# HKPolyU-UAV/bluerov2

Measured on AMD Instinct MI355X. Metric: NMPC RTI solves/s (N=20, 12 states / 4 inputs), batch 4096 per GPU, higher is better.
Workload: dtype f64; 1 GPU; BASELINE.json configs[1]: batch=4096 independent BlueROV2 NMPC instances per GPU, N=20, Ts=0.05 s, circle reference window advancing one row per step, per-instance x0 noise (seed 1), nominal parameters, default options (qp_early_exit=1: exact equality-constrained shortcut when no bound is active); batch_per_gpu=4096, N=20, parallelism=single GPU

## Files before the change

### bluerov2_amd/csrc/nmpc_api.hip

```cpp
#include <hip/hip_runtime.h>

#include <algorithm>
#include <cstddef>
#include <cstdio>
#include <cstdlib>
#include <cmath>
#include <cstring>
#include <string>
#include <atomic>
#include <chrono>
#include <vector>

#include "host_common.hpp"
#include "nmpc_device.hpp"
#include "select_device.hpp"
#include "wrench_source.hpp"

using namespace brov;

#define kTickMailboxMaxBatch 64

static thread_local std::string g_err;
extern "C" const char* brov_last_error(void) { return g_err.c_str(); }

// ... 69 lines not shown
    WrenchSource wr;
    bool cand_set = false;
    int cand_kind = 0;
    bool dump_lin = false;
    int* lines = nullptr;
    DeviceAllocs mem;
    hipStream_t last_stream = nullptr;
    bool timing = false;
    hipEvent_t ev[3] = {nullptr, nullptr, nullptr};
    bool ev_valid = false;
    int last_family = 0;
    int cus = 256;
    double* ws = nullptr;
    int32_t* counter = nullptr;
    unsigned win_count = 0;
    int win_blocks = 0, win_L = 0;
    double* ws_split = nullptr;
    int alt_blocks = 0, alt_L = 0;
    int prep_path = 0;
    unsigned long long* dbg = nullptr;
    std::vector<double> ts_host;
    double W0_host[16] = {0};
    bool has_W0 = false;
    double* tsv = nullptr;
    double* wst = nullptr;
    int32_t* sched = nullptr;
    unsigned sched_tick = 0;
    TickChannel tick;
    bool pit_ran = false;
    int32_t* pit_done = nullptr;
    DevKnobs k;
};

static int env_int(const char* name, int dflt) { const char* v = getenv(name); return v ? atoi(v) : dflt; }
static DevKnobs read_knobs() {
    DevKnobs k;
    k.robust_pivot = env_int("BROV_ROBUST_PIVOT", 1);
    if (const char* v = getenv("BROV_ROBUST_KKT_MAX")) k.robust_kkt_max = atof(v);
    k.partial_refactor = env_int("BROV_PARTIAL_REFACTOR", 1) != 0;
    k.mail_early = env_int("BROV_DEV_NO_EARLY_RECORD", 0) == 0;
    k.split_resident = env_int("BROV_SPLIT_RESIDENT", 1) != 0;
    k.pit = env_int("BROV_PIT", 1);
    k.split_parallel = env_int("BROV_SPLIT_PARALLEL", 1) != 0;
    k.pit_try = env_int("BROV_PIT_TRY", 1) != 0;
    k.pit_light = env_int("BROV_PIT_LIGHT", 1) != 0;
    k.tick_mailbox = env_int("BROV_TICK_MAILBOX", 1) != 0;
    k.tick_bulk = env_int("BROV_TICK_BULK", 1) != 0;
    k.tick_zerocopy = env_int("BROV_TICK_ZEROCOPY", 1) != 0;
    k.sched = env_int("BROV_SCHED", 1) != 0;
    k.force_windowed = env_int("BROV_DEV_FORCE_WINDOWED", 0) != 0;
    k.fused_waves = env_int("BROV_DEV_FUSED_WAVES", 0);
    k.lds_pad = env_int("BROV_DEV_LDS_PAD", 0);
    k.closed_loop_fused = env_int("BROV_CLOSED_LOOP_FUSED", 1) != 0;
    k.tick_breakdown = env_int("BROV_TICK_BREAKDOWN", 0) != 0;
    k.no_resident = env_int("BROV_DEV_NO_RESIDENT", 0) != 0;
    k.win_blocks = env_int("BROV_DEV_WIN_BLOCKS", 0);
    k.pit_rounds = env_int("BROV_PIT_ROUNDS", 1) != 0;
    k.win_long = env_int("BROV_DEV_WIN_LONG", 0) != 0;
    return k;
}
extern "C" int brov_dev_reload_knobs(brov_solver* s) {
    if (!s) return BROV_ERR_ARG;
    const DevKnobs at_create = s->k;
    s->k = read_knobs();
    s->k.force_windowed = at_create.force_windowed; s->k.no_resident = at_create.no_resident;
    s->k.win_blocks = at_create.win_blocks; s->k.pit_rounds = at_create.pit_rounds;
    return BROV_OK;
}

extern "C" void brov_default_opts(brov_opts* o, int N, double Ts) {
    static const double W[16] = {300, 480, 200, 10, 10, 200, 40, 40, 10, 10, 10, 10, 1, 1, 0.1, 0.05};
    std::memset(o, 0, sizeof(*o));
    o->N = N;
    o->Ts = Ts;
    for (int j = 0; j < 16; j++) o->W[j] = W[j];
    for (int j = 0; j < 12; j++) o->We[j] = W[j];
    for (int j = 0; j < 4; j++) { o->lbu[j] = -50.0; o->ubu[j] = 50.0; }
    o->qp_iter_max = 50;
    o->qp_tol_mu = 1e-7;
    o->qp_tol_stat = 1e-9;
    o->qp_early_exit = 1;
    o->kernel_path = BROV_PATH_AUTO;
    o->on_failure = BROV_ON_FAILURE_RESTART;
}

static const char* opts_problem(const brov_opts* o) {
    if (o->N < 1 || o->N > BROV_MAX_N) return "N out of range";
    if (!(o->Ts > 0.0) || !(o->Ts < 1e6)) return "Ts must be positive and finite";
    if (o->kernel_path < 0 || o->kernel_path > 2) return "kernel_path must be BROV_PATH_AUTO / _STREAMING / _FUSED";
    if (o->on_failure < 0 || o->on_failure > 1) return "on_failure must be BROV_ON_FAILURE_KEEP / _RESTART";
    for (int j = 0; j < 16; j++)
        if (!(o->W[j] >= 0.0) || !(o->W[j] < 1e300)) return "stage weights must be finite and >= 0";
    for (int j = 12; j < 16; j++)
        if (!(o->W[j] > 0.0)) return "input weights W[12..15] must be > 0 (strictly convex QP)";
    for (int j = 0; j < 12; j++)
        if (!(o->We[j] >= 0.0) || !(o->We[j] < 1e300)) return "terminal weights must be finite and >= 0";
    for (int j = 0; j < 4; j++)
        if (!(o->lbu[j] < o->ubu[j]) || !(o->lbu[j] > -1e300) || !(o->ubu[j] < 1e300)) return "input bounds need lbu < ubu, both finite";
    if (o->qp_iter_max < 1) return "qp_iter_max must be >= 1";
    if (!(o->qp_tol_mu > 0.0) || !(o->qp_tol_stat > 0.0)) return "qp tolerances must be > 0";
    return nullptr;
}

static void invalidate_preparation(brov_solver* s) { if (s && s->prep_path == 2) s->prep_path = 3; }
static void forget_traj_window(brov_solver* s) { s->yref_view = nullptr; s->traj_line = -1; }
static bool serves_fused(const brov_solver* s) { return fused_supported(s->N) && !s->k.force_windowed; }
static bool serves_windowed_ticks(const brov_solver* s) { return s->ws != nullptr && !windowed_is_resident(s->win_L) && s->alt_L == 0; }

static bool general_grid(const brov_solver* s) { return !s->ts_host.empty() || s->has_W0; }
static int upload_grid(brov_solver* s) {
    if (!general_grid(s)) return BROV_OK;
    const int N = s->N;
    if (!s->tsv) {
        if (int rc = s->mem.alloc(&s->tsv, (size_t)N, g_err)) return rc;
        if (int rc = s->mem.alloc(&s->wst, (size_t)(N + 1) * 16, g_err)) return rc;
    }
    std::vector<double> ts(N), w((size_t)(N + 1) * 16, 0.0);
    for (int i = 0; i < N; i++) {
        ts[i] = s->ts_host.empty() ? s->opts.Ts : s->ts_host[i];
// ... 529 lines not shown
enum { FAM_STREAMING = 0, FAM_FUSED, FAM_WINDOWED };
struct SolvePlan {
    int family = FAM_STREAMING;
    bool split_ok = false;
    int rti_split = 0;
    double* ws = nullptr;
    int64_t ws_stride = 0;
    int win_L = 0, win_blocks = 0;
    int pit = 0, pit_blocks = 0;
    int prep_path = 1;
};
static SolvePlan plan_solve(const brov_solver* s, int rti_phase) {
    SolvePlan p;
    const bool lds = s->opts.kernel_path != BROV_PATH_STREAMING, fused_h = serves_fused(s);
    const bool may_split = lds && !s->dump_lin && s->k.split_resident;
    const bool split_fused = may_split && fused_h && s->ws_split != nullptr;
    p.split_ok = split_fused || (may_split && !fused_h && s->ws != nullptr && windowed_is_resident(s->win_L) && s->win_blocks == s->B);
    const bool split = p.split_ok && (rti_phase == 1 || (rti_phase == 2 && s->prep_path == 2));
    p.prep_path = split ? 2 : 1;
    p.ws = s->ws; p.win_L = s->win_L; p.win_blocks = s->win_blocks;
    if (split && split_fused) { p.ws = s->ws_split; p.win_L = s->N; p.win_blocks = s->B; }
    p.ws_stride = p.win_L ? (int64_t)windowed_ws_doubles(s->N, p.win_L) : 0;
    if (!lds || (rti_phase != 0 && !split)) return p;
    if (fused_h && !split) { p.family = FAM_FUSED; return p; }
    if (!p.ws) return p;
    p.family = FAM_WINDOWED;
    p.rti_split = rti_phase;
    p.pit_blocks = p.win_blocks;
    bool pit = false;
    if (s->k.pit && rti_phase == 2) {
        pit = s->k.split_parallel && pit_supported(s->N, p.win_L);
    } else if (s->k.pit && rti_phase == 0 && !s->dump_lin) {
        if (s->alt_L) {
            p.win_L = s->alt_L; p.win_blocks = s->alt_blocks; p.ws_stride = (int64_t)windowed_ws_doubles(s->N, s->alt_L);
            p.pit_blocks = s->B;
        }
        pit = pit_supported(s->N, p.win_L);
    }
    p.pit = pit ? s->k.pit : 0;
    return p;
}

static DevParams make_params(const brov_solver* s, const SolvePlan& plan, const LaunchInputs* in = nullptr) {
    static const LaunchInputs none;
    if (!in) in = &none;
    DevParams P;
    std::memset(&P, 0, sizeof P);
    P.B = s->B; P.N = s->N;
    P.qp_iter_max = s->opts.qp_iter_max; P.early_exit = s->opts.qp_early_exit;
    P.on_failure = s->opts.on_failure; P.dump_lin = s->dump_lin ? 1 : 0;
    P.robust_kkt_max = s->k.robust_kkt_max;
    P.robust_pivot = s->k.robust_pivot;
    P.partial_refactor = s->k.partial_refactor;
    P.Ts = s->opts.Ts; P.tol_mu = s->opts.qp_tol_mu; P.tol_stat = s->opts.qp_tol_stat;
    for (int j = 0; j < 16; j++) P.W[j] = s->opts.W[j];
    for (int j = 0; j < 12; j++) P.We[j] = s->opts.We[j];
    for (int j = 0; j < 4; j++) { P.lbu[j] = s->opts.lbu[j]; P.ubu[j] = s->opts.ubu[j]; }
    P.x0 = in->x0 ? in->x0 : s->x0;
    P.yref = in->yref ? in->yref : (s->yref_shared ? shared_window(s) : s->yref);
    P.yref_stride = s->yref_shared ? 0 : (int64_t)(s->N + 1) * 16;
    P.par = in->par ? in->par : s->par;
    P.par_rp = s->dist6 ? s->par_rp : nullptr;
    P.tsv = general_grid(s) ? s->tsv : nullptr;
    P.sched = s->k.sched ? s->sched : nullptr;
    P.sched_stride = sched_buffer_ints_host(s->B);
    P.sched_r = (int)(s->sched_tick % 3); P.sched_w = (int)((s->sched_tick + 1) % 3); P.sched_z = (int)((s->sched_tick + 2) % 3);
    P.wst = general_grid(s) ? s->wst : nullptr;
    P.x = s->x; P.u = s->u; P.pi = s->pi; P.lam = s->lam;
    P.BA = s->BA; P.bvec = s->bvec; P.kktp = s->kktp;
    P.Ks = s->Ks; P.Kt = s->Kt; P.Mt = s->Mt; P.Pb = s->Pb; P.kff = s->kff; P.vhat = s->vhat; P.ipm = s->ipm;
    P.dxb = s->dxb; P.cst = s->cst; P.res = s->res;
    P.mail = in->mail; P.mail_flag = in->mail_flag; P.mail_seq = in->mail_seq;
    P.mail_early = s->k.mail_early;
    P.counter = s->counter + 32 * (s->win_count & 1u);
    P.counter_next = s->counter + 32 * ((s->win_count + 1u) & 1u);
    P.ws = plan.ws; P.ws_stride = plan.ws_stride; P.win_L = plan.win_L; P.win_blocks = plan.win_blocks;
    P.rti_split = plan.rti_split; P.pit_blocks = plan.pit_blocks;
    if (plan.pit) { P.pit = plan.pit; P.pit_done = s->pit_done; P.pit_try = s->k.pit_try; P.pit_light = s->k.pit_light; }
    P.dbg = s->dbg;
    return P;
}
static void launch_lds(brov_solver* s, const DevParams& P, int family, hipStream_t st) {
    if (family == FAM_FUSED) launch_fused(P, st, s->k);
    else { launch_windowed(P, st, s->k); s->win_count++; }
    s->pit_ran = P.pit != 0;
    s->last_family = family;
    s->last_stream = st;
}
static void time_mark(brov_solver* s, int k, hipStream_t st) {
    if (s->timing) { hipEventRecord(s->ev[k], st); s->ev_valid = s->ev_valid || k == 2; }
}
struct PlantInLaunch { double dt; int substeps; double *xlog, *ulog; };
static int launch_ticks(brov_solver* s, int family, int n, int64_t row_stride_doubles, int32_t* status_log, const PlantInLaunch* plant,
                        hipStream_t st) {
    if (int rc = order_behind_last(s, st)) return rc;
    DevParams P = make_params(s, plan_solve(s, 0));
    P.sched = nullptr;
    P.ticks = n; P.tick_yref = row_stride_doubles; P.tick_status = status_log;
    if (plant) {
        P.plant_pp = s->pplant; P.plant_rp = plant_rp(s); P.plant_rp_stride = plant_rp_stride(s); P.plant_substeps = plant->substeps; P.plant_dt = plant->dt;
        P.x0_rw = s->x0; P.plant_xlog = plant->xlog; P.plant_ulog = plant->ulog;
    }
    time_mark(s, 0, st); time_mark(s, 1, st);
    launch_lds(s, P, family, st); s->prep_path = 0;
    time_mark(s, 2, st);
    if (row_stride_doubles > 0) {
// ... 563 lines not shown
```

### bluerov2_amd/csrc/nmpc_device.hpp

```cpp
#pragma once
#include <string>
#include <hip/hip_runtime.h>
#include <stdint.h>

#include "../../include/bluerov2_nmpc.h"

namespace brov {

struct DevParams {
    int32_t B, N;
    int32_t qp_iter_max, early_exit;
    int32_t pit;
    int32_t pit_light;
    int32_t pit_try;
    int32_t pit_blocks;
    int32_t* pit_done;
    double robust_kkt_max;
    int32_t partial_refactor, robust_pivot;
    int32_t rti_split;
    int32_t on_failure, dump_lin;
    double Ts, tol_mu, tol_stat;
    double W[16], We[12], lbu[4], ubu[4];
    const double* x0;
    const double* yref;
    int64_t yref_stride;
    const double* par;
    const double* par_rp;
    double* x;
    double* u;
    double* pi;
    double* lam;
    double* BA;
    double* bvec;
    double* kktp;
    double* Ks;
    double* Kt;
    double* Mt;
    double* Pb;
    double* kff;
    double* vhat;
    double* ipm;
    double* dxb;
    const double* cst;
    const double* tsv;
    const double* wst;
    brov_result* res;
    brov_result* mail;
    int32_t* mail_flag;
    int32_t mail_seq;
    int32_t mail_early;
    double* ws;
    int64_t ws_stride;
    int32_t* counter;
    int32_t* counter_next;
    int32_t win_L, win_blocks;
    int32_t* sched;
    int32_t sched_stride, sched_r, sched_w, sched_z;
    int32_t ticks;
    int64_t tick_yref;
    int32_t* tick_status;
    const double* plant_pp;
    const double* plant_rp;
    int32_t plant_rp_stride, plant_substeps;
    double plant_dt;
    double* x0_rw;
    double* plant_xlog;
    double* plant_ulog;
    unsigned long long* dbg;
};

struct DevKnobs {
    double robust_kkt_max = 1e6;
    int robust_pivot = 1, partial_refactor = 1, mail_early = 1, split_resident = 1, pit = 1, split_parallel = 1, pit_try = 1, pit_light = 1;
    int tick_mailbox = 1, tick_bulk = 1, tick_zerocopy = 1, sched = 1, force_windowed = 0, fused_waves = 0, lds_pad = 0, tick_breakdown = 0, closed_loop_fused = 1;
    int no_resident = 0, win_blocks = 0, pit_rounds = 1;
    int win_long = 0;
};

enum { IPM_V = 0, IPM_TL, IPM_TU, IPM_LL, IPM_LU, IPM_GAM, IPM_RT, IPM_DVA, IPM_ACT, IPM_NARR };

int sched_buffer_ints_host(int B);
int prepare_kernels_on_device(std::string* why);
void launch_linearise(const DevParams& P, hipStream_t st);
void launch_qp(const DevParams& P, hipStream_t st);
void launch_fused(const DevParams& P, hipStream_t st, const DevKnobs& k);
bool fused_supported(int N);
void launch_windowed(const DevParams& P, hipStream_t st, const DevKnobs& k);
void lds_kernel_info(int N, int win_L, bool windowed, int32_t info[4], const DevKnobs& k);
bool pit_supported(int N, int win_L);
bool windowed_is_resident(int win_L);
int windowed_stage_count(int N, int B, int cus, const DevKnobs& k);
int windowed_blocks(int B, int L, int cus, const DevKnobs& k);
size_t windowed_ws_doubles(int N, int L);
bool split_resident_horizon(int N);
int pit_rounds_stages(int N, int B, int cus, const DevKnobs& k);
void launch_window(const double* traj, int rows, const int* lines, int line0, int B, int N, int ncols, double* out, hipStream_t st);
void launch_plant(double* x0, const brov_result* res, const double* pplant, const double* prp, int rp_stride, int B, double dt, int substeps,
                  double* xlog, double* ulog, hipStream_t st);
void launch_candidates(int kind, const double* p0, const double* p1, const double* phase, double t0, double dt, int B, int N,
                       double* out, hipStream_t st);

struct WrenchGen {
    int mode = 0;
    int rows = 0;
    const double* w = nullptr;
    const double* tab = nullptr;
    const double* gain = nullptr;
    unsigned long long seed = 0;
    double scale = 6.0, phase0 = 0.0, dphi = 0.125, tz_div = 3.0;
};
void launch_plant_wrench(double* x0, const brov_result* res, const double* pplant, const double* prp, int rp_stride, int B, double dt, int substeps,
                         double* xlog, double* ulog, const WrenchGen& g, long long tick, double* wlog , hipStream_t st);
void launch_wrench_eval(const WrenchGen& g, int B, long long tick, double* out , hipStream_t st);
void launch_gather_cols(const double* src, int B, int src_stride, int col0, int ncols, double* dst , hipStream_t st);

}
```

### bluerov2_amd/csrc/qp/qp_body.hpp

```cpp
#pragma once

namespace brov {

#define DBG_STAMP(slot) do { if (P.dbg && lane == 0) {                                                                          \
        P.dbg[(size_t)b * 8 + (slot)] = __builtin_readcyclecounter();                                                           \
        if ((slot) == 0) P.dbg[(size_t)P.B * 8 + (size_t)b * 8 + 7] = __builtin_amdgcn_s_memrealtime();                        \
        if ((slot) == 0) P.dbg[(size_t)P.B * 8 + (size_t)b * 8 + 5] = ((unsigned long long)__builtin_amdgcn_s_getreg(63508) << 32) | __builtin_amdgcn_s_getreg(63492); \
        if ((slot) == 6) P.dbg[(size_t)P.B * 8 + (size_t)b * 8 + 6] = __builtin_amdgcn_s_memrealtime(); } } while (0)
#ifdef BROV_DBG_IPM
#define IPM_T(k) do { const unsigned long long t_ = __builtin_readcyclecounter(); ipm_t[k] += t_ - ipm_last; ipm_last = t_; } while (0)
#else
#define IPM_T(k) do { } while (0)
#endif

#ifdef BROV_DBG_LIN
#define LIN_T(k) do { __builtin_amdgcn_sched_barrier(0); lin_t[k] = __builtin_readcyclecounter(); __builtin_amdgcn_sched_barrier(0); } while (0)
#else
#define LIN_T(k) do { } while (0)
#endif

template <int LDS, class IT = Inst, bool DF = false, bool LONGV = false>
__device__ __forceinline__ void qp_body(const DevParams& P, IT& I, int b, double lin_part, bool lin_nan, Win* W = nullptr,
                                        bool pre_ok = true, bool pre_illc = false) {
    constexpr bool EL = (LDS == 1 || LDS == 2);
    const double* __restrict__ cst = P.cst;
    const int lane = I.lane, N = I.NT, nv = I.nv;
    DBG_STAMP(1);
    const int rg = I.rg;

    double* x_it = P.x + (size_t)b * (N + 1) * 12;
    double* u_it = P.u + (size_t)b * N * 4;
    double* pi_it = P.pi + (size_t)b * N * 12;
    double* lam_it = P.lam + (size_t)b * N * 8;
    double* V = I.ipm + (size_t)IPM_V * nv;
    double* TL = I.ipm + (size_t)IPM_TL * nv;
    double* TU = I.ipm + (size_t)IPM_TU * nv;
    double* LL = I.ipm + (size_t)IPM_LL * nv;
    double* LU = I.ipm + (size_t)IPM_LU * nv;
    double* GAM = I.ipm + (size_t)IPM_GAM * nv;
    double* RT = I.ipm + (size_t)IPM_RT * nv;
    double* DVA = I.ipm + (size_t)IPM_DVA * nv;
    double* ACT = I.ipm + (size_t)IPM_ACT * nv;
    const double* GRAD = EL ? (const double*)I.kff : (const double*)DVA;
    auto rd_vhat = [&](int j) -> double { if constexpr (EL) return I.lds_vhat[j]; else return I.vhat[j]; };
    auto wr_vhat = [&](int j, double v) { if constexpr (EL) I.lds_vhat[j] = v; else I.vhat[j] = v; };
    auto rd_dxb = [&](int j) -> double { if constexpr (EL) return I.lds_dxb[j]; else return I.dxb[j]; };
    auto rd_grad = [&](int j) -> double { if constexpr (EL) return I.lds_kff[j]; else return GRAD[j]; };

    double x0v[3], xiv[3];
    {
        const double* x0 = P.x0 + (size_t)b * 12;
#pragma unroll
        for (int r = 0; r < 3; r++) { x0v[r] = x0[rg + 4 * r]; xiv[r] = I.x[rg + 4 * r]; }
    }

    double ureg[2] = {0.0, 0.0};
    if constexpr (EL) {
#pragma unroll
        for (int t = 0; t < 2; t++)
            if (lane + 64 * t < nv) ureg[t] = I.u[lane + 64 * t];
    }
    int status = 0, iters = 0;
    double mu = 0.0, rho = 0.0;
    bool early = false, polished = false, use_vhat = false;
    int sched_p = -1;
    bool ok = pre_ok;
    constexpr bool PART = EL || LDS >= 3;
    bool illc0 = pre_illc;
    bool split0 = false;
    if constexpr (EL) split0 = I.ckpt > 0;
    if constexpr (EL) { if (split0) {
        BwdState S;
        wave_fence();
        bwd_init<true, LDS>(I, S);
#pragma clang loop unroll(disable)
        for (int ph = 0; ph < 2; ph++) {
            if (ph == 1) {
                if (I.ckpt == 0) break;
                double* ck = I.Kt;
#pragma unroll
                for (int r = 0; r < 3; r++) { ck[r * 64 + lane] = S.P[r]; ck[192 + r * 64 + lane] = S.pv[r]; }
            }
            bwd_chunk<true, LDS, false, true>(I, S, ph == 0 ? N : I.ckpt, ph == 0 ? I.ckpt : 0);
        }
        ok = S.ok;
        illc0 = S.illc;
    } }
    if constexpr (LDS < 3) { if (!split0) ok = riccati_backward<true, LDS, false, true>(I, &illc0); }
    d4 d0;
    double kkt = 0.0;
    {
#pragma unroll
        for (int r = 0; r < 3; r++) {
            d0[r] = x0v[r] - xiv[r];
            kkt_upd(kkt, d0[r]);
        }
        d0[3] = 0.0;
        double part = lin_part;
        bool nanp = lin_nan;
        if (kkt != kkt) nanp = true;
        kkt = wave_max(fmax(part, (kkt != kkt) ? 0.0 : kkt));
        if (__ballot(nanp) != 0ull) kkt = __builtin_nan("");
    }
    constexpr bool ROB = LDS != 2;
    bool robust = false, robust_ok = false;
    if constexpr (ROB) {
        robust_ok = kkt <= P.robust_kkt_max || P.robust_pivot == 3;
        if ((__ballot(illc0) != 0ull && P.robust_pivot && robust_ok) || P.robust_pivot == 2) {
            robust = true;
            I.ckpt = 0;
            ok = sw_backward<true, LDS, true, true>(I, W);
        }
    }
    DBG_STAMP(2);
    const double lbc = EL ? cst[32 + (lane & 3)] : 0.0, ubc = EL ? cst[36 + (lane & 3)] : 0.0;
    if (__ballot(!ok) != 0ull) {
        status = BROV_STATUS_QP_FAILURE;
    } else {
        sw_forward<LDS>(I, W, d0, cst);
        DBG_STAMP(3);
        bool feas = true;
        if constexpr (LDS >= 3) {
            feas = W->feas;
        } else if constexpr (EL) {
#pragma unroll
            for (int t = 0; t < 2; t++) {
                const int j = lane + 64 * t;
                if (j < nv) {
                    const double vj = rd_vhat(j), lb = lbc - ureg[t], ub = ubc - ureg[t];
                    if (!(vj >= lb && vj <= ub)) feas = false;
                }
            }
        } else {
            for (int j = lane; j < nv; j += 64) {
                const int m = j & 3;
                const double vj = rd_vhat(j), lb = cst[32 + m] - I.u[j], ub = cst[36 + m] - I.u[j];
                if (!(vj >= lb && vj <= ub)) feas = false;
            }
        }
        const bool allfeas = (__ballot(!feas) == 0ull);
        if (allfeas && P.early_exit) {
            early = true;
        } else {
#ifdef BROV_DBG_IPM
            unsigned long long ipm_t[8] = {0, 0, 0, 0, 0, 0, 0, 0}, ipm_last = __builtin_readcyclecounter();
#endif
            constexpr bool CACHE = (LDS >= 3) && !LONGV;
            constexpr int kIpmT = EL ? 2 : ((LDS == 0 || LONGV) ? 16 : 8);
            using Vec = IpmVec<EL ? 1 : (CACHE ? 2 : 0), kIpmT>;
            Vec vV{{}, V}, vTL{{}, TL}, vTU{{}, TU}, vLL{{}, LL}, vLU{{}, LU}, vDVA{{}, DVA},
                vDLL{{}, GAM}, vDLU{{}, RT},
                vACT{{}, ACT};
#define IPM_FOR(t, j) _Pragma("unroll") for (int t = 0; t < kIpmT; t++) if (const unsigned j = (unsigned)lane + 64u * t; j < (unsigned)nv)
#define IPM_PRE(arr, expr)                                                                     \
            double arr[CACHE ? kIpmT : 1];                                                         \
            if constexpr (CACHE) {                                                                 \
                _Pragma("unroll") for (int t = 0; t < kIpmT; t++) {                                \
                    const unsigned j = ((unsigned)lane + 64u * t < (unsigned)nv) ? (unsigned)lane + 64u * t : 0u; \
                    arr[t] = (expr);                                                               \
                }                                                                                  \
            }
            auto set_act = [&](int t, int j, double v) __attribute__((always_inline)) { if constexpr (CACHE) ACT[j] = v; else vACT.set(t, j, v); };
#define GROUP_LANE int lane_g_ = I.lane; asm volatile("v_mov_b32 %0, %0" : "+v"(lane_g_)); const int lane = lane_g_
            const int mI = lane & 3;
            double lbI = cst[32 + mI], ubI = cst[36 + mI], wuI = cst[12 + mI];
            asm volatile("" : "+v"(lbI), "+v"(ubI), "+v"(wuI));
            const double rdI = P.Ts * wuI;
            auto rd_el = [&](unsigned j) __attribute__((always_inline)) -> double {
// ... 367 lines not shown

    constexpr int UX = EL ? 5 : 4, UU = EL ? 2 : 4;
    const double* vfin = (early || EL || use_vhat) ? I.vhat : V;
    const int nxe = (N + 1) * 12;
    double cost = 0.0;
    bool wrote_u0 = false;
    double u0v = 0.0;
    if (status == BROV_STATUS_SUCCESS || status == BROV_STATUS_MAXITER) {
        if (!early && !polished) {
            sw_rollout<LDS>(I, W, d0, vfin);
        }
        DBG_STAMP(4);
        if constexpr (LDS >= 3) {
            if (W->nan) {
                status = BROV_STATUS_NAN;
            } else {
                win_adjoint_commit<LDS == 4>(P, I, *W, b, vfin, early, cost, u0v, P.mail != nullptr && P.mail_early != 0,
                                             [&](double cost_lane, double u0_lane) __attribute__((always_inline)) { emit_record(cost_lane, u0_lane, true); });
                wrote_u0 = true;
            }
            DBG_STAMP(5);
        } else {
        double xpre[UX], ypre[UX], urpre[UU];
        double wxpre[LDS == 1 ? UX : 1], wupre[LDS == 1 ? UU : 1];
        if constexpr (EL) {
#pragma unroll
            for (int t = 0; t < UX; t++) {
                const int j = lane + 64 * t;
                const int jj = j < nxe ? j : 0;
                const int i = div12(jj), c = jj - i * 12;
                xpre[t] = x_it[jj];
                ypre[t] = I.yref[(size_t)i * 16 + c];
                if constexpr (LDS == 1) wxpre[t] = cst[(i == N) ? 16 + c : c];
            }
#pragma unroll
            for (int t = 0; t < UU; t++) {
                const int j = lane + 64 * t;
                const int jj = j < nv ? j : 0;
                urpre[t] = I.yref[(size_t)(jj >> 2) * 16 + 12 + (jj & 3)];
                if constexpr (LDS == 1) wupre[t] = cst[12 + (jj & 3)];
            }
        }
        auto copy_pi = [&]() __attribute__((always_inline)) {
            double pv5[5];
#pragma unroll
            for (int t = 0; t < 5; t++) pv5[t] = I.lds_kt[lane + 64 * t < N * 12 ? lane + 64 * t : 0];
#pragma unroll
            for (int t = 0; t < 5; t++) asm volatile("" : "+v"(pv5[t]));
#pragma unroll
            for (int t = 0; t < 5; t++)
                if (lane + 64 * t < N * 12) pi_it[lane + 64 * t] = pv5[t];
        };
        const bool late = DF && EL && early && P.mail != nullptr;
        if (!(EL && polished) && !late) sw_adjoint<true, LDS>(I, W, vfin, DVA, pi_it);
        DBG_STAMP(5);
        bool nanv = false;
        double vvp[EL ? UU : 1], djp[EL ? UX : 1];
        if constexpr (EL) {
#pragma unroll
            for (int t = 0; t < UU; t++) vvp[t] = rd_vhat(lane + 64 * t < nv ? lane + 64 * t : 0);
#pragma unroll
            for (int t = 0; t < UX; t++) djp[t] = rd_dxb(lane + 64 * t < nxe ? lane + 64 * t : 0);
#pragma unroll
            for (int t = 0; t < UU; t++) nanv = nanv || !(vvp[t] == vvp[t]);
#pragma unroll
            for (int t = 0; t < UX; t++) nanv = nanv || !(djp[t] == djp[t]);
        } else {
            for (int j = lane; j < nv; j += 64) {
                const double vj = vfin[j];
                if (!(vj == vj)) nanv = true;
            }
            for (int j = lane; j < nxe; j += 64) {
                const double dj = rd_dxb(j);
                if (!(dj == dj)) nanv = true;
            }
        }
        if (__ballot(nanv) != 0ull) {
            status = BROV_STATUS_NAN;
        } else {
            for (int j0 = lane; j0 < nv; j0 += 64 * UU) {
                double uo[UU], vv[UU], gg[UU], ur[UU];
#pragma unroll
                for (int t = 0; t < UU; t++) {
                    const int j = j0 + 64 * t;
                    const bool in = j < nv;
                    const int jj = in ? j : 0;
                    uo[t] = (EL && j0 == lane && t < 2) ? ureg[t] : u_it[jj];
                    vv[t] = EL ? ((j0 == lane) ? vvp[EL ? t : 0] : rd_vhat(jj)) : vfin[jj];
                    gg[t] = early ? 0.0 : rd_grad(jj);
                    ur[t] = (EL && j0 == lane) ? urpre[t] : I.yref[(size_t)(jj >> 2) * 16 + 12 + (jj & 3)];
                }
#pragma unroll
                for (int t = 0; t < UU; t++) {
                    const int j = j0 + 64 * t;
                    if (j < nv) {
                        const int i = j >> 2, m = j & 3;
                        lam_it[i * 8 + m] = gg[t] > 0 ? gg[t] : 0.0;
                        lam_it[i * 8 + 4 + m] = gg[t] < 0 ? -gg[t] : 0.0;
                        const double un = uo[t] + vv[t];
                        u_it[j] = un;
                        if (j < 4) { P.res[b].u0[j] = un; u0v = un; }
                        const double e = un - ur[t];
                        const double wgt = (LDS == 1 && j0 == lane) ? wupre[LDS == 1 ? t : 0] : cst[12 + m];
                        const double sw = (IT::kGrid || (LDS == 0 && I.wst)) ? I.wst[(size_t)i * 16 + 12 + m] : P.Ts * wgt;
                        cost += 0.5 * sw * e * e;
                    }
                }
            }
            wrote_u0 = true;
            if constexpr (EL) {
                if (!late) copy_pi();
            }
            for (int j0 = lane; j0 < nxe; j0 += 64 * UX) {
                double xo[UX], dj[UX], yr[UX];
#pragma unroll
                for (int t = 0; t < UX; t++) {
                    const int j = j0 + 64 * t;
                    const int jj = j < nxe ? j : 0;
                    const int i = div12(jj), c = jj - i * 12;
                    xo[t] = (EL && j0 == lane) ? xpre[t] : x_it[jj];
                    dj[t] = (EL && j0 == lane) ? djp[EL ? t : 0] : rd_dxb(jj);
                    yr[t] = (EL && j0 == lane) ? ypre[t] : I.yref[(size_t)i * 16 + c];
                }
#pragma unroll
                for (int t = 0; t < UX; t++) {
                    const int j = j0 + 64 * t;
                    if (j < nxe) {
                        const int i = div12(j), c = j - i * 12;
                        const double xn = xo[t] + dj[t];
                        x_it[j] = xn;
                        const double e = xn - yr[t];
                        const double wgt = (LDS == 1 && j0 == lane) ? wxpre[LDS == 1 ? t : 0] : cst[(i == N) ? 16 + c : c];
                        const double sw = (IT::kGrid || (LDS == 0 && I.wst)) ? I.wst[(size_t)i * 16 + c] : ((i == N) ? wgt : P.Ts * wgt);
                        cost += 0.5 * sw * e * e;
                    }
                }
            }
        }
        if constexpr (DF && EL) {
            if (late && status == BROV_STATUS_SUCCESS) {
                emit_record(cost, u0v, wrote_u0);
                sw_adjoint<true, LDS>(I, W, vfin, DVA, pi_it);
                copy_pi();
            } else if (late) {
            }
        }
        }
    }
    if (status != BROV_STATUS_SUCCESS && status != BROV_STATUS_MAXITER) {
        const double* x0 = P.x0 + (size_t)b * 12;
        const double xl = x0[lane < 12 ? lane : 0];
        const bool restart = P.on_failure == BROV_ON_FAILURE_RESTART && __ballot(!(fabs(xl) < 1e300)) == 0ull;
        for (int j = lane; j < nv; j += 64) {
            const int i = j >> 2, m = j & 3;
            const double e = u_it[j] - I.yref[(size_t)i * 16 + 12 + m];
            cost += 0.5 * ((IT::kGrid || (LDS == 0 && I.wst)) ? I.wst[(size_t)i * 16 + 12 + m] : P.Ts * cst[12 + m]) * e * e;
            if (restart) { u_it[j] = 0.0; lam_it[i * 8 + m] = 0.0; lam_it[i * 8 + 4 + m] = 0.0; }
        }
        for (int j = lane; j < nxe; j += 64) {
            const int i = j / 12, c = j - i * 12;
            const double e = x_it[j] - I.yref[(size_t)i * 16 + c];
            cost += 0.5 * ((IT::kGrid || (LDS == 0 && I.wst)) ? I.wst[(size_t)i * 16 + c] : ((i == N) ? cst[16 + c] : P.Ts * cst[c])) * e * e;
            if (restart) { x_it[j] = x0[c]; if (i < N) pi_it[j] = 0.0; }
        }
    }
    if (!emitted) emit_record(cost, u0v, wrote_u0);
#ifdef BROV_SCHED_TICKET_LATE
    if (sched_p == -2) sched_p = sched_ticket(P, b);
#endif
    sched_note(P, b, sched_p);
    I.ran_loop = !early;
    DBG_STAMP(6);
}


struct LaneCst { double Wr[4], Wer[3], lbm, ubm, Wq, Weq, Wuq; };
__device__ __forceinline__ LaneCst load_lane_cst(const double* __restrict__ cst, int lane) {
    const int rg = lane >> 4;
    LaneCst c;
#pragma unroll
    for (int r = 0; r < 4; r++) c.Wr[r] = cst[rg + 4 * r];
#pragma unroll
    for (int r = 0; r < 3; r++) c.Wer[r] = cst[16 + rg + 4 * r];
    c.lbm = cst[32 + rg];
    c.ubm = cst[36 + rg];
    const int cq = (lane >> 2) < NX ? (lane >> 2) : NX - 1;
    c.Wq = cst[cq];
    c.Weq = cst[16 + cq];
    c.Wuq = cst[12 + ((lane >> 2) & 3)];
    return c;
}
__device__ __forceinline__ void setup_inst(const DevParams& P, Inst& I, int b, int lane, const LaneCst* pre = nullptr, size_t yoff = 0) {
    const int N = P.N, nv = 4 * N;
    const double* __restrict__ cst = P.cst;
    I.lane = lane; I.rg = lane >> 4; I.cl = lane & 15; I.N = N; I.nv = nv;
// ... 38 lines not shown
```

### bluerov2_amd/csrc/qp/sweeps.hpp

```cpp
#pragma once

namespace brov {

template <int LDS> constexpr int kLdsDist = LDS == 2 ? 1 : 2;

struct BwdIn {
    d4 ba;
    d4 bv;
    double xv[3], yv[3];
    double rtv, gm;
    double ks, mt;
};

struct Ba1Off { int off[3], str; };
template <bool FACTOR, int LDS, bool STEP0 = false, class IT = Inst>
__device__ __forceinline__ BwdIn load_bwd(const IT& I, int i, const double* gam, const double* rt, const Ba1Off* b1 = nullptr) {
    BwdIn s;
    s.ba = get_ba<LDS>(I, i);
    const int ig = I.i0 + i;
    if constexpr (FACTOR && LDS != 0) {
        if (b1) {
            const lds_f64* t = I.lds_ba + lmul(i, b1->str);
            s.bv = d4{t[b1->off[0]], t[b1->off[1]], t[b1->off[2]], 0.0};
        } else {
// ... 49 lines not shown
        if (FACTOR) {
#pragma unroll
            for (int r = 0; r < 3; r++) pv[r] = (cl == 0) ? pv[r] : 0.0;
        }
    }
    S.P = P; S.pv = pv; S.ok = true;
}

struct SolveV { double m[12], ks[4], pb, q, rt; };
template <int LDS>
__device__ __forceinline__ void bwd_solve_v(const Inst& I, BwdState& S) {
    static_assert(LDS != 0, "LDS-resident kernels only");
    const int rg = I.rg, cl = I.cl, N = I.N;
    const int k = I.lane & 15;
    const bool rowx = k < NX, ecol = k < 3;
    const int oc = k >= 3 ? k - 3 : 0, kx = rowx ? k : NX - 1, ku = k & 3;
    const double* rt = I.ipm + (size_t)IPM_RT * I.nv;
    store_vec12_lds(I.lds_tr, S.pv, rg, cl);
    double pcur = I.lds_tr[kx];
    if (I.lane < 16)
    pipelined<(LDS == 3 ? 3 : kLdsDist<LDS>), SolveV>(N, [&](int kk) {
        const int i = N - 1 - kk, ig = I.i0 + i;
        SolveV s;
        const lds_f64* col = I.lds_ba + i * kBaStage + oc;
#pragma unroll
        for (int r = 0; r < 12; r++) s.m[r] = col[r * kBaStride];
        const double* kt = I.Ks + (size_t)ig * 64 + k;
#pragma unroll
        for (int t = 0; t < 4; t++) s.ks[t] = kt[16 * t];
        s.pb = I.Pb[(size_t)ig * 12 + kx];
        s.q = I.lds_q[i * 12 + kx];
        s.rt = rt[ig * 4 + ku];
        return s; },
                                     [&](int kk, const SolveV& in) {
        const int i = N - 1 - kk;
        const double l = in.pb + pcur;
        double d0 = 0.0, d1 = 0.0, d2 = 0.0, d3 = 0.0;
        fmac_bc12(d0, d1, d2, d3, l, in.m[0], in.m[1], in.m[2], in.m[3], in.m[4], in.m[5], in.m[6], in.m[7], in.m[8], in.m[9], in.m[10], in.m[11]);
        const double g = (ecol ? l : (d0 + d1) + (d2 + d3)) + (rowx ? in.q : in.rt);
        double t0 = 0.0, t1 = 0.0;
        fmac_bc4(t0, t1, g, in.ks[0], in.ks[1], in.ks[2], in.ks[3]);
        const double t = t0 + t1;
        lds_f64* kp = rowx ? I.lds_tr + 16 : I.lds_kff + i * 4 + ku;
        *kp = -t;
        pcur = g + t;
    });
    lds_f64* tp = (rowx && I.lane < 16) ? I.lds_tr + k : I.lds_tr + 16;
    *tp = pcur;
    const lds_f64* tl = I.lds_tr + rg;
    S.pv = d4{tl[0], tl[4], tl[8], 0.0};
}

template <bool FACTOR, int LDS, bool STORE_IPM = true, bool STEP0 = false, bool ROBUST = false, class IT = Inst, bool ACC = false>
__device__ __forceinline__ void bwd_chunk(const IT& I, BwdState& S, int hi = -1, int lo = 0) {
    PitAcc* const acc = &S.acc;
    static_assert(!ACC || (FACTOR && LDS == 3 && !ROBUST && !STORE_IPM), "ACC: the factor sweeps of rti_pit_kernel");
    if constexpr (!FACTOR && LDS != 0) {
        bwd_solve_v<LDS>(I, S);
        return;
    }
    const int lane = I.lane, rg = I.rg, cl = I.cl, N = hi < 0 ? I.N : hi;
    const double* gam = I.ipm + (size_t)IPM_GAM * I.nv;
    const double* rt = I.ipm + (size_t)IPM_RT * I.nv;
    BwdIn nx;
    d4& P = S.P;
    d4& pv = S.pv;
    bool& ok = S.ok;
    bool& illc = S.illc;
    const d4 z4 = {0, 0, 0, 0};
    const unsigned mk_col0 = cl == 0 ? ~0u : 0u;
    constexpr bool kMaskPvAtUse = (LDS == 1 || LDS == 2);
    const double col0f = cl == 0 ? 1.0 : 0.0;
    d4 diagm;
#pragma unroll
    for (int r = 0; r < 3; r++) diagm[r] = (rg + 4 * r == cl) ? I.Ts * I.Wr[r] : 0.0;
    diagm[3] = (12 + rg == cl) ? I.Ts * I.Wr[3] : 0.0;
    constexpr bool kR6 = (LDS == 1 || LDS == 2) && !ROBUST;
    constexpr bool kR6Z = kR6 && LDS == 1;
    const int pR = rg, pC = cl & 3;
    const double sR0 = pR == 0 ? 1.0 : 0.0, sR1 = pR == 1 ? 1.0 : 0.0, nR2 = pR == 2 ? -1.0 : 0.0, nR3 = pR == 3 ? -1.0 : 0.0;
    const double nC0 = pC == 0 ? -1.0 : 0.0, nC1 = pC == 1 ? -1.0 : 0.0, cC2 = pC == 2 ? 1.0 : 0.0, cC3 = pC == 3 ? 1.0 : 0.0;
    const double nE00 = (pR == 0 && pC == 0) ? -1.0 : 0.0, nE01 = (pR + pC == 1) ? -1.0 : 0.0, nE11 = (pR == 1 && pC == 1) ? -1.0 : 0.0;
    d4 dgz = diagm;
    dgz[0] = lane == 0 ? 0.0 : diagm[0];
    lds_f64* const kt_st0 = (LDS != 0 && cl < NX) ? I.lds_kt + rg * NX + cl : I.lds_tr + 16;
    const int kt_ststr = (cl < NX) ? kKtStage : 0;
    constexpr int kKffCol = kR6 ? 12 : 0;
    lds_f64* const kf_st0 = (LDS != 0 && cl == kKffCol) ? I.lds_kff + rg : I.lds_tr + 16;
    const int kf_ststr = (cl == kKffCol) ? 4 : 0;
    lds_f64* ktp = kt_st0 + lmul(N - 1, kt_ststr);
    lds_f64* kfp = kf_st0 + lmul(N - 1, kf_ststr);
    unsigned long long illm = 0;
    Ba1Off b1o;
    if constexpr (LDS != 0) {
        const int bvrel = (int)(I.lds_bv - I.lds_ba);
#pragma unroll
        for (int r = 0; r < 3; r++) b1o.off[r] = cl == 0 ? bvrel + rg + 4 * r : I.ba_off[r];
        b1o.str = cl == 0 ? NX : I.ba_str;
    }
    const Ba1Off* const b1 = kR6 ? &b1o : nullptr;
    auto stage = [&](int i, const BwdIn& in, auto&& mid) __attribute__((always_inline)) {
        d4 qr;
#pragma unroll
        for (int r = 0; r < 3; r++) qr[r] = LDS ? in.xv[r] : I.Ts * I.Wr[r] * (in.xv[r] - in.yv[r]);
        qr[3] = (!LDS && STEP0) ? I.Ts * I.Wr[3] * in.rtv : in.rtv;
        d4 dg = diagm;
        if constexpr (IT::kGrid && LDS != 0 && FACTOR) {
            dg[0] = (rg == cl) ? in.yv[0] : 0.0; dg[1] = (rg + 4 == cl) ? in.yv[1] : 0.0; dg[2] = (rg + 8 == cl) ? in.yv[2] : 0.0;
            dg[3] = (12 + rg == cl) ? in.mt : 0.0;
        }
        if constexpr (!LDS) {
            if (I.wst) {
                const double* ws = I.wst + (size_t)i * 16 + rg;
                const double w0 = ws[0], w1 = ws[4], w2 = ws[8], w3 = ws[12];
                qr[0] = w0 * (in.xv[0] - in.yv[0]); qr[1] = w1 * (in.xv[1] - in.yv[1]); qr[2] = w2 * (in.xv[2] - in.yv[2]);
                if (STEP0) qr[3] = w3 * in.rtv;
                dg[0] = (rg == cl) ? w0 : 0.0; dg[1] = (rg + 4 == cl) ? w1 : 0.0; dg[2] = (rg + 8 == cl) ? w2 : 0.0;
                dg[3] = (12 + rg == cl) ? w3 : 0.0;
            }
        }
        if (FACTOR) {
// ... 148 lines not shown
            } else if constexpr (kR6) {
                pn = tn1(ks, g[3], g);
                pn[3] = ks;
            } else {
                const d4 kf = tn1(mt, g[3], z4);
                pn = tn1(ks, g[3], g);
                pn[3] = kf[0];
            }
            if (STORE_IPM) {
                I.Ks[(size_t)(I.i0 + i) * 64 + lane] = kR6Z ? ((cl < NX) ? ks : -msel) : xt2;
            }
            if constexpr (LDS) {
                if constexpr (kR6) {
                    *ktp = ks; ktp -= kt_ststr;
                } else {
                    lds_f64* t = (cl < NX) ? I.lds_kt + i * kKtStage + rg * NX + cl : I.lds_zero;
                    *t = (cl < NX) ? ks : 0.0;
                }
            } else {
                d4 KtT = tn1(H[3], -mt, z4);
                double* kt = I.Kt + (size_t)i * 192;
                kt[lane] = KtT[0]; kt[64 + lane] = KtT[1]; kt[128 + lane] = KtT[2];
            }
            if constexpr (LDS) {
                if constexpr (kR6) {
                    *kfp = pn[3]; kfp -= kf_ststr;
                } else {
                    lds_f64* kp = (cl == 0) ? I.lds_kff + i * 4 + rg : I.lds_zero;
                    *kp = (cl == 0) ? -pn[3] : 0.0;
                }
            } else if (cl == 0) {
                I.kff[i * 4 + rg] = -pn[3];
            }
            if constexpr (ACC) {
                d4 R = Racc;
                const double bPsi = R[0];
                R[0] = (rg == 0) ? acc->Psi[0] : R[0];
                const d4 MZt = tn1(mt, R[3], z4);
                const double MZ0 = kR6Z ? -MZt[0] : MZt[0];
                I.Ks[(size_t)(I.i0 + i) * 64 + lane] = MZ0;
                const double kffb = dpp_f64<0x150>(kR6Z ? pn[3] : -pn[3]);
                const double Xg = (cl < NX) ? MZ0 : ((cl == NX) ? kffb : 0.0);
                d4 Gn = tn1(Xg, R[3], acc->G);
                Gn[3] += (rg == 0) ? bPsi : 0.0;
                acc->G = Gn;
                d4 Pn = tn1(ks, R[3], d4{R[0], R[1], R[2], 0.0});
                Pn[3] = 0.0;
                acc->Psi = Pn;
            }
            P = S;
#pragma unroll
            for (int r = 0; r < 3; r++) pv[r] = kMaskPvAtUse ? pn[r] : blend(mk_col0, pn[r], 0.0);
            pv[3] = 0.0;
        } else {
            mid();
            d4 l;
#pragma unroll
            for (int r = 0; r < 4; r++) l[r] = in.bv[r] + pv[r];
            d4 g = tn<3>(in.ba, l, qr);
            const d4 gC = {g[0], g[1], g[2], 0.0};
            d4 pn = tn1(in.ks, g[3], gC);
            if constexpr (LDS) I.lds_kff[i * 4 + rg] = -pn[3]; else if (cl == 0) I.kff[i * 4 + rg] = -pn[3];
            pv = pn;
            pv[3] = 0.0;
        }
    };
    if constexpr (LDS) {
        const int cnt = N - lo;
        if constexpr (LDS == 2) {
            pipelined<kLdsDist<LDS>, BwdIn>(cnt, [&](int k) { return load_bwd<FACTOR, LDS, STEP0>(I, N - 1 - k, gam, rt, b1); },
                                [&](int k, const BwdIn& in) { stage(N - 1 - k, in, [] {}); });
        } else {
            pipelined_mid<kLdsDist<LDS>, BwdIn>(cnt, [&](int k) { return load_bwd<FACTOR, LDS, STEP0>(I, N - 1 - k, gam, rt, b1); },
                                [&](int k, const BwdIn& in, auto&& issue) { stage(N - 1 - k, in, issue); });
        }
    } else {
        nx = load_bwd<FACTOR, LDS, STEP0>(I, N - 1, gam, rt);
        for (int i = N - 1; i >= 0; i--) {
            const BwdIn in = nx;
            if (i > 0) nx = load_bwd<FACTOR, LDS, STEP0>(I, i - 1, gam, rt);
            stage(i, in, [] {});
        }
    }
    if constexpr (FACTOR && kR6) illc = illc | (illm != 0ull);
}

template <bool FACTOR, int LDS, bool STORE_IPM = true, bool STEP0 = false, bool ROBUST = false, class IT = Inst>
__device__ bool riccati_backward(const IT& I, bool* illc = nullptr) {
    BwdState S;
    wave_fence();
    bwd_init<FACTOR, LDS>(I, S);
    bwd_chunk<FACTOR, LDS, STORE_IPM, STEP0, ROBUST>(I, S);
    if (illc) *illc = S.illc;
    return S.ok;
}

template <int LDS, class IT = Inst>
__device__ __forceinline__ bool riccati_backward_tries(const IT& I, bool part, const double (&kff0)[2], bool& illc) {
    static_assert(LDS == 1 || LDS == 2, "fused kernels");
    wave_fence();
    BwdState S;
    if (part) {
#pragma unroll
        for (int t = 0; t < 2; t++) {
            const int j = I.lane + 64 * t;
            I.lds_kff[j < I.nv ? j : 0] = kff0[t];
        }
        const double* ck = I.Kt;
#pragma unroll
        for (int r = 0; r < 3; r++) { S.P[r] = ck[r * 64 + I.lane]; S.pv[r] = ck[192 + r * 64 + I.lane]; }
        S.P[3] = 0.0; S.pv[3] = 0.0; S.ok = true;
    } else {
        bwd_init<true, LDS>(I, S);
    }
    bwd_chunk<true, LDS, true, false>(I, S, part ? I.ckpt : I.N, 0);
    illc = S.illc;
    return S.ok;
}

struct FwdIn { d4 kt, bat, bb; double kf; };
template <int LDS>
__device__ __forceinline__ FwdIn load_fwd(const Inst& I, int i) {
    FwdIn s;
    if constexpr (LDS) {
        const lds_f64* t = I.lds_ba + lmul(i, I.kt_str);
        s.kt = d4{t[I.kt_off[0]], t[I.kt_off[1]], t[I.kt_off[2]], 0.0};
    } else {
        s.kt = load_tile3(I.Kt + (size_t)i * 192, I.lane);
    }
    s.bat = get_bat<LDS>(I, i);
    s.bb = get_bv<LDS>(I, i);
    if constexpr (LDS) s.kf = I.lds_kff[i * 4 + I.rg]; else s.kf = I.kff[i * 4 + I.rg];
    return s;
}

__device__ __forceinline__ double quad_sum(double v) {
    v += dpp_f64<0xB1>(v);
    v += dpp_f64<0x4E>(v);
    return v;
}
struct FwdV { double m[12], b4[4], cv; };
__device__ __forceinline__ FwdV load_fwd_v(const lds_f64* mrow, const lds_f64* klo, const lds_f64* brow, const lds_f64* cvec) {
    FwdV s;
#pragma unroll
    for (int c = 0; c < 3; c++) s.m[c] = klo[c];
// ... 188 lines not shown
            const double qd = IT::kGrid ? in.wq : ((I.i0 + i + 1 == I.NT) ? I.Weq : I.Ts * I.Wq);
            const double pic = fma(qd, in.dxc, in.qc + gq);
            *pp = pic; pp -= pstr;
            const lds_f64* pr = I.lds_kt + i * NX + 4 * q3;
            const double p0 = pr[0], p1 = pr[1], p2 = pr[2], p3 = pr[3];
            __builtin_amdgcn_sched_barrier(0);
            const double m0 = ecol ? e0 : in.m[0], m1 = ecol ? e1 : in.m[1], m2 = ecol ? e2 : in.m[2], m3 = ecol ? e3 : in.m[3];
            double acc = m0 * p0;
            acc = fma(m1, p1, acc); acc = fma(m2, p2, acc); acc = fma(m3, p3, acc);
            acc = colx ? acc : 0.0;
            const double G = quad_sum(acc);
            *gp = fma(IT::kGrid ? in.wr : rd, in.vm, in.rm + G); gp -= gstr;
            gq = G;
        });
        lds_f64* tpark = rowx ? I.lds_tr + c : I.lds_tr + 16;
        *tpark = gq;
        const lds_f64* tl = I.lds_tr + rg;
        atpi = d4{tl[0], tl[4], tl[8], 0.0};
        return;
    }
    const d4 z4 = {0, 0, 0, 0};
    auto stage = [&](int i, const AdjIn& in) __attribute__((always_inline)) {
        d4 pi;
        double wq[3], wr;
        if (I.wst) {
            const double* ws = I.wst + (size_t)(i + 1) * 16 + rg;
            wq[0] = ws[0]; wq[1] = ws[4]; wq[2] = ws[8];
            wr = I.wst[(size_t)i * 16 + 12 + rg];
        } else {
#pragma unroll
            for (int r = 0; r < 3; r++) wq[r] = (I.i0 + i + 1 == I.NT) ? I.Wer[r] : I.Ts * I.Wr[r];
            wr = I.Ts * I.Wr[3];
        }
#pragma unroll
        for (int r = 0; r < 3; r++) pi[r] = wq[r] * (in.dx[r] + in.xn[r] - in.yn[r]) + atpi[r];
        pi[3] = 0.0;
        if (COMMIT) store_vec12(pi_out + (size_t)i * 12, pi, rg, cl);
        d4 G = tn<3>(in.ba, pi, z4);
        const double rd = wr;
        if (cl == 0) garr[i * 4 + rg] = rd * in.v + rd * (in.u - in.ur) + G[3];
        atpi = G;
    };
    pipelined<3, AdjIn>(N, [&](int k) { return load_adj<LDS>(I, N - 1 - k, varr); },
                        [&](int k, const AdjIn& in) { stage(N - 1 - k, in); });
}
template <bool COMMIT, int LDS, class IT = Inst>
__device__ void adjoint(const IT& I, const double* varr, double* garr, double* pi_out) {
    wave_fence();
    d4 atpi = {0, 0, 0, 0};
    adj_chunk<COMMIT, LDS>(I, atpi, varr, garr, pi_out);
    wave_fence();
}

}
```

Measured before the change: 5.754 million solves/s.

## Split adjoint sweep into four parallel segments seeded by Riccati checkpoints

During the factorising backward Riccati sweep, the (P, pv) state is checkpointed at segment boundaries spaced N/4 apart. In the early-exit path, the serial adjoint recursion over N stages is replaced by four independent segments, one per row group, each seeded from its checkpoint. This shortens the dependent chain of the adjoint pass at the cost of extra global stores during the backward sweep and some redundant lanes. It is only used for LDS==1 non-grid kernels with N>=12, and is disabled when the robust or ill-conditioned KKT path is taken.

```diff
diff --git a/bluerov2_amd/csrc/nmpc_api.hip b/bluerov2_amd/csrc/nmpc_api.hip
--- a/bluerov2_amd/csrc/nmpc_api.hip
+++ b/bluerov2_amd/csrc/nmpc_api.hip
@@ -145,6 +145,7 @@
     k.fused_waves = env_int("BROV_DEV_FUSED_WAVES", 0);
     k.lds_pad = env_int("BROV_DEV_LDS_PAD", 0);
     k.closed_loop_fused = env_int("BROV_CLOSED_LOOP_FUSED", 1) != 0;
+    k.adj_segments = env_int("BROV_ADJ_SEGMENTS", 1) != 0;
     k.tick_breakdown = env_int("BROV_TICK_BREAKDOWN", 0) != 0;
     k.no_resident = env_int("BROV_DEV_NO_RESIDENT", 0) != 0;
     k.win_blocks = env_int("BROV_DEV_WIN_BLOCKS", 0);
@@ -158,6 +159,7 @@
     s->k = read_knobs();
     s->k.force_windowed = at_create.force_windowed; s->k.no_resident = at_create.no_resident;
     s->k.win_blocks = at_create.win_blocks; s->k.pit_rounds = at_create.pit_rounds;
+    s->k.adj_segments = at_create.adj_segments;
     return BROV_OK;
 }
 
@@ -793,6 +795,7 @@
     P.robust_kkt_max = s->k.robust_kkt_max;
     P.robust_pivot = s->k.robust_pivot;
     P.partial_refactor = s->k.partial_refactor;
+    P.adj_segments = s->k.adj_segments;
     P.Ts = s->opts.Ts; P.tol_mu = s->opts.qp_tol_mu; P.tol_stat = s->opts.qp_tol_stat;
     for (int j = 0; j < 16; j++) P.W[j] = s->opts.W[j];
     for (int j = 0; j < 12; j++) P.We[j] = s->opts.We[j];
diff --git a/bluerov2_amd/csrc/nmpc_device.hpp b/bluerov2_amd/csrc/nmpc_device.hpp
--- a/bluerov2_amd/csrc/nmpc_device.hpp
+++ b/bluerov2_amd/csrc/nmpc_device.hpp
@@ -17,6 +17,7 @@
     int32_t* pit_done;
     double robust_kkt_max;
     int32_t partial_refactor, robust_pivot;
+    int32_t adj_segments;
     int32_t rti_split;
     int32_t on_failure, dump_lin;
     double Ts, tol_mu, tol_stat;
@@ -72,7 +73,7 @@
 struct DevKnobs {
     double robust_kkt_max = 1e6;
     int robust_pivot = 1, partial_refactor = 1, mail_early = 1, split_resident = 1, pit = 1, split_parallel = 1, pit_try = 1, pit_light = 1;
-    int tick_mailbox = 1, tick_bulk = 1, tick_zerocopy = 1, sched = 1, force_windowed = 0, fused_waves = 0, lds_pad = 0, tick_breakdown = 0, closed_loop_fused = 1;
+    int tick_mailbox = 1, tick_bulk = 1, tick_zerocopy = 1, sched = 1, force_windowed = 0, fused_waves = 0, lds_pad = 0, tick_breakdown = 0, closed_loop_fused = 1, adj_segments = 1;
     int no_resident = 0, win_blocks = 0, pit_rounds = 1;
     int win_long = 0;
 };
diff --git a/bluerov2_amd/csrc/qp/qp_body.hpp b/bluerov2_amd/csrc/qp/qp_body.hpp
--- a/bluerov2_amd/csrc/qp/qp_body.hpp
+++ b/bluerov2_amd/csrc/qp/qp_body.hpp
@@ -69,6 +69,9 @@
     bool illc0 = pre_illc;
     bool split0 = false;
     if constexpr (EL) split0 = I.ckpt > 0;
+    constexpr bool SEG = LDS == 1 && !IT::kGrid;
+    int segLs = 0;
+    if constexpr (SEG) segLs = (P.adj_segments && N >= 12) ? (N + 3) >> 2 : 0;
     if constexpr (EL) { if (split0) {
         BwdState S;
         wave_fence();
@@ -81,12 +84,12 @@
 #pragma unroll
                 for (int r = 0; r < 3; r++) { ck[r * 64 + lane] = S.P[r]; ck[192 + r * 64 + lane] = S.pv[r]; }
             }
-            bwd_chunk<true, LDS, false, true>(I, S, ph == 0 ? N : I.ckpt, ph == 0 ? I.ckpt : 0);
+            bwd_chunk<true, LDS, false, true>(I, S, ph == 0 ? N : I.ckpt, ph == 0 ? I.ckpt : 0, segLs);
         }
         ok = S.ok;
         illc0 = S.illc;
     } }
-    if constexpr (LDS < 3) { if (!split0) ok = riccati_backward<true, LDS, false, true>(I, &illc0); }
+    if constexpr (LDS < 3) { if (!split0) ok = riccati_backward<true, LDS, false, true>(I, &illc0, segLs); }
     d4 d0;
     double kkt = 0.0;
     {
@@ -114,6 +117,14 @@
     }
     DBG_STAMP(2);
     const double lbc = EL ? cst[32 + (lane & 3)] : 0.0, ubc = EL ? cst[36 + (lane & 3)] : 0.0;
+    SegPre segp = {};
+    if constexpr (SEG) {
+        if (robust || !(kkt <= P.robust_kkt_max)) segLs = 0;
+        if (segLs > 0) {
+            wave_fence();
+            segp = adj_seg_request(I, cst);
+        }
+    }
     if (__ballot(!ok) != 0ull) {
         status = BROV_STATUS_QP_FAILURE;
     } else {
@@ -587,7 +598,12 @@
                 if (lane + 64 * t < N * 12) pi_it[lane + 64 * t] = pv5[t];
         };
         const bool late = DF && EL && early && P.mail != nullptr;
-        if (!(EL && polished) && !late) sw_adjoint<true, LDS>(I, W, vfin, DVA, pi_it);
+        bool seg = false;
+        if constexpr (SEG) seg = early && segLs > 0;
+        if (!(EL && polished) && !late) {
+            if constexpr (SEG) { if (seg) adj_seg(I, segLs, segp); }
+            if (!seg) sw_adjoint<true, LDS>(I, W, vfin, DVA, pi_it);
+        }
         DBG_STAMP(5);
         bool nanv = false;
         double vvp[EL ? UU : 1], djp[EL ? UX : 1];
@@ -675,7 +691,8 @@
         if constexpr (DF && EL) {
             if (late && status == BROV_STATUS_SUCCESS) {
                 emit_record(cost, u0v, wrote_u0);
-                sw_adjoint<true, LDS>(I, W, vfin, DVA, pi_it);
+                if constexpr (SEG) { if (seg) adj_seg(I, segLs, segp); }
+                if (!seg) sw_adjoint<true, LDS>(I, W, vfin, DVA, pi_it);
                 copy_pi();
             } else if (late) {
             }
diff --git a/bluerov2_amd/csrc/qp/sweeps.hpp b/bluerov2_amd/csrc/qp/sweeps.hpp
--- a/bluerov2_amd/csrc/qp/sweeps.hpp
+++ b/bluerov2_amd/csrc/qp/sweeps.hpp
@@ -125,8 +125,9 @@
 }
 
 template <bool FACTOR, int LDS, bool STORE_IPM = true, bool STEP0 = false, bool ROBUST = false, class IT = Inst, bool ACC = false>
-__device__ __forceinline__ void bwd_chunk(const IT& I, BwdState& S, int hi = -1, int lo = 0) {
+__device__ __forceinline__ void bwd_chunk(const IT& I, BwdState& S, int hi = -1, int lo = 0, int capLs = 0) {
     PitAcc* const acc = &S.acc;
+    constexpr bool kCap = FACTOR && LDS == 1 && STEP0 && !ROBUST && !IT::kGrid && !ACC;
     static_assert(!ACC || (FACTOR && LDS == 3 && !ROBUST && !STORE_IPM), "ACC: the factor sweeps of rti_pit_kernel");
     if constexpr (!FACTOR && LDS != 0) {
         bwd_solve_v<LDS>(I, S);
@@ -140,6 +141,11 @@
     d4& pv = S.pv;
     bool& ok = S.ok;
     bool& illc = S.illc;
+    int capm = 0, capnext = -1;
+    if constexpr (kCap) {
+        if (capLs > 0) capm = 3 * capLs < N ? 3 : (2 * capLs < N ? 2 : (capLs < N ? 1 : 0));
+        capnext = capm > 0 ? capm * capLs : -1;
+    }
     const d4 z4 = {0, 0, 0, 0};
     const unsigned mk_col0 = cl == 0 ? ~0u : 0u;
     constexpr bool kMaskPvAtUse = (LDS == 1 || LDS == 2);
@@ -394,6 +400,15 @@
 #pragma unroll
             for (int r = 0; r < 3; r++) pv[r] = kMaskPvAtUse ? pn[r] : blend(mk_col0, pn[r], 0.0);
             pv[3] = 0.0;
+            if constexpr (kCap) {
+                if (i == capnext) {
+                    double* cp = I.Kt + capm * 384;
+#pragma unroll
+                    for (int r = 0; r < 3; r++) { cp[r * 64 + lane] = P[r]; cp[192 + r * 64 + lane] = pv[r]; }
+                    capm--;
+                    capnext = capm > 0 ? capnext - capLs : -1;
+                }
+            }
         } else {
             mid();
             d4 l;
@@ -428,11 +443,11 @@
 }
 
 template <bool FACTOR, int LDS, bool STORE_IPM = true, bool STEP0 = false, bool ROBUST = false, class IT = Inst>
-__device__ bool riccati_backward(const IT& I, bool* illc = nullptr) {
+__device__ bool riccati_backward(const IT& I, bool* illc = nullptr, int capLs = 0) {
     BwdState S;
     wave_fence();
     bwd_init<FACTOR, LDS>(I, S);
-    bwd_chunk<FACTOR, LDS, STORE_IPM, STEP0, ROBUST>(I, S);
+    bwd_chunk<FACTOR, LDS, STORE_IPM, STEP0, ROBUST>(I, S, -1, 0, capLs);
     if (illc) *illc = S.illc;
     return S.ok;
 }
@@ -727,4 +742,60 @@
     wave_fence();
 }
 
-}
+struct SegPre { dbl2 pr[6]; double pc, wq, weq; };
+__device__ __forceinline__ SegPre adj_seg_request(const Inst& I, const double* __restrict__ cst) {
+    const int k = I.lane & 15, kx = k < NX ? k : NX - 1, s = I.rg < 2 ? I.rg : 2;
+    SegPre r;
+    const double* row = I.Kt + (2 + 2 * s) * 192 + 16 * kx;
+    const dbl2* row2 = (const dbl2*)row;
+#pragma unroll
+    for (int t = 0; t < 6; t++) r.pr[t] = row2[t];
+    r.pc = row[192];
+    r.wq = cst[kx];
+    r.weq = cst[16 + kx];
+    return r;
+}
+struct AdjS { double m[12], dxc, qc; };
+__device__ __forceinline__ void adj_seg(const Inst& I, int Ls, const SegPre& pre) {
+    wave_fence();
+    const int N = I.N, s = I.rg, k = I.lane & 15;
+    const bool rowx = k < NX, ecol = k < 3;
+    const int oc = k >= 3 ? k - 3 : 0, kx = rowx ? k : NX - 1;
+    const int lo = lmul(s, Ls);
+    const int hi = lo + Ls < N ? lo + Ls : N;
+    const int ntr = hi - lo - 1;
+    lds_f64* const park = I.lds_tr + 16;
+    const double dxh = I.lds_dxb[lmul(hi, NX) + kx], qh = I.lds_q[lmul(hi, NX) + kx];
+    double d0 = pre.pc, d1 = 0.0, d2 = 0.0, d3 = 0.0;
+    fmac_bc12(d0, d1, d2, d3, dxh, pre.pr[0][0], pre.pr[0][1], pre.pr[1][0], pre.pr[1][1], pre.pr[2][0], pre.pr[2][1], pre.pr[3][0],
+              pre.pr[3][1], pre.pr[4][0], pre.pr[4][1], pre.pr[5][0], pre.pr[5][1]);
+    double picur = hi == N ? fma(pre.weq, dxh, qh) : (d0 + d1) + (d2 + d3);
+    lds_f64* pp = rowx ? I.lds_kt + lmul(hi - 1, NX) + k : park;
+    const int pstr = rowx ? NX : 0;
+    *pp = picur; pp -= pstr;
+    const double qd = I.Ts * pre.wq;
+    const lds_f64* col0 = I.lds_ba + lmul(hi - 1, kBaStage) + oc;
+    const lds_f64* dx0 = I.lds_dxb + lmul(hi - 1, NX) + kx;
+    const lds_f64* q0 = I.lds_q + lmul(hi - 1, NX) + kx;
+    pipelined<kLdsDist<1>, AdjS>(Ls - 1, [&](int kk) {
+        AdjS in;
+        const lds_f64* col = col0 - lmul(kk, kBaStage);
+#pragma unroll
+        for (int r = 0; r < 12; r++) in.m[r] = col[r * kBaStride];
+        in.dxc = dx0[-lmul(kk, NX)];
+        in.qc = q0[-lmul(kk, NX)];
+        return in; },
+                                 [&](int kk, const AdjS& in) {
+        double g0 = 0.0, g1 = 0.0, g2 = 0.0, g3 = 0.0;
+        fmac_bc12(g0, g1, g2, g3, picur, in.m[0], in.m[1], in.m[2], in.m[3], in.m[4], in.m[5], in.m[6], in.m[7], in.m[8], in.m[9], in.m[10], in.m[11]);
+        const double gq = ecol ? picur : (g0 + g1) + (g2 + g3);
+        const double pic = fma(qd, in.dxc, in.qc + gq);
+        const bool act = kk < ntr;
+        picur = act ? pic : picur;
+        lds_f64* st = act ? pp : park;
+        *st = picur; pp -= pstr;
+    });
+    wave_fence();
+}
+
+}
```

Result: slower. 5.680 million solves/s (-1.3%).
